# kmkolasinski/tfrecords-reader

Measured on AMD Instinct MI355X. Metric: GiB/s + examples/s device-resident TFRecord->Feature decode, 1/2/4/8 GPU, higher is better.
Workload: dtype u8; 1 GPU; C4 directory (configs[4]) of 256 files, C1-shaped (int64 label + 12 B bytes_list id) records, 524288 +-50 % per file (default_rng(1000+f)), spec CRC-32C; this rank's LPT share (256 files) resident in HBM; records_per_gpu=134295581, framed_bytes_per_gpu=7906235019, parallelism=file-sharded x1 (LPT by bytes, no collective on the data path), batches_per_gpu=4, batch_bytes_max=1976558779, streams=2, tpl_groups_missed=0

## Files before the change

### tfrecords-reader_amd/csrc/tfrg_capi.cpp

```cpp
#include <hip/hip_runtime.h>
#include <stdlib.h>
#include <string.h>

#include <algorithm>
#include <map>
#include <numeric>
#include <string>
#include <unordered_map>
#include <vector>

#include "../../include/tfrg.h"
#include "crc32c.h"
#include "tfrg_dense.h"
#include "tfrg_frame.h"
#include "tfrg_internal.h"
#include "tfrg_learn.h"

namespace tfrg {
void set_error(const std::string& s);

#define HIP_TRY(expr)                                                              \
  do {                                                                             \
    hipError_t e_ = (expr);                                                        \
    if (e_ != hipSuccess) {                                                        \
// ... 27 lines not shown
  template <class T>
  T* as() const {
    return reinterpret_cast<T*>(p);
  }
};

constexpr uint32_t kMissCap = 1u << 16;

}

using namespace tfrg;

struct Offsets {
  const uint64_t* s64 = nullptr;
  const uint64_t* e64 = nullptr;
  const uint32_t* s32 = nullptr;
  const uint32_t* e32 = nullptr;
  uint32_t first = 0;
  uint32_t mode = kOffU64;
};

struct tfrg_ctx {
  int device = 0;
  hipStream_t own_stream = nullptr;
  hipStream_t last_stream = nullptr;
  uint32_t lane_max = 2048;
  uint32_t wave_stage = 0xffffffffu;
  uint64_t record_bound = 0;
  uint64_t call_bound = 0;
  int num_cus = 256;
  uint32_t cu_lds = 65536;
  int tpl_stage = 1;
  uint32_t tpl_gpw = 0;
  DBuf crc_tab, consts;
  DBuf ht, key_hash, key_off, key_blob, key_slot, slot_kind, key_w, krec;
  uint32_t n_keys = 0, n_slots = 0, ht_mask = 0;
  DBuf in_bytes, in_start, in_end;
  DBuf status, aux, verdict, order, count, loc, rs, slot_base, totals, kind_totals;
  DBuf ident;
  size_t ident_n = 0;
  DBuf i64, f32, b_off, b_len, big_list, slow_list, miss, info, tsum, crc_rec, crc_base, crc_part;
  DBuf dq, dq_cnt;
  DBuf lmask, rlist;
  DBuf bdata, boff64, blb, bbig;
  bool materialized = false;
  bool tsum_dirty = true;
  uint32_t info_slot = 0;
  bool info_clean = false;
  uint32_t n = 0;
  uint64_t cap_hint = 0;
  hipEvent_t order_ev = nullptr;
  hipEvent_t dense_ev[2] = {nullptr, nullptr};
  int dense_nt = 0;
  uint64_t nbytes = 0;
  uint64_t cap_i64 = 0, cap_f32 = 0, cap_b = 0;
  bool have_result = false;
  bool rs_complete = false;
  std::unordered_map<std::string, uint32_t> key_id;
  std::vector<int32_t> key_slot_h;
  DBuf tpl;
  uint32_t n_tpl = 0;
  uint32_t tpl_w = 0;
  size_t tpl_img_off = 0;
  uint32_t tpl_img_words = 0;
  uint32_t tpl_tab_words = 0;
  std::vector<uint32_t> tpl_h;
// ... 32 lines not shown
    uint64_t cap_in;
    uint64_t bound;
    uint32_t n, flags;
    hipStream_t st;
  } last{};
  Offsets last_off{};
  uint32_t index_chunk = kIndexChunkDefault;
  DBuf fr_tab, fr_dev;
  void* fr_pin = nullptr;
  size_t fr_pin_cap = 0;
  uint32_t poison[4] = {0xffffffffu, 0xffffffffu, 0xffffffffu, 0xffffffffu};
};

extern "C" {

int tfrg_ctx_create(int device, tfrg_ctx** out) {
  *out = nullptr;
  int ndev = 0;
  HIP_TRY(hipGetDeviceCount(&ndev));
  if (device < 0 || device >= ndev) {
    set_error("bad device index");
    return TFRG_E_ARG;
  }
  HIP_TRY(hipSetDevice(device));
  tfrg_ctx* c = new tfrg_ctx();
  c->device = device;
  if (const char* e = getenv("TFRG_TEMPLATES")) c->tpl_on = atoi(e) != 0;
  if (const char* e = getenv("TFRG_SPEC")) c->spec_on = atoi(e) != 0;
  if (const char* e = getenv("TFRG_TPL_STAGE")) c->tpl_stage = atoi(e);
  if (const char* e = getenv("TFRG_TPL_GPW")) {
    const int v = atoi(e);
    if (v == 2 || v == 4 || v == 8) c->tpl_gpw = (uint32_t)v;
  }
  if (const char* e = getenv("TFRG_OPTIMISTIC")) c->optimistic_on = atoi(e) != 0;
  if (const char* e = getenv("TFRG_WALK_BESIDE")) c->walk_beside = atoi(e) != 0;
  if (const char* e = getenv("TFRG_WALK_BLOCKS")) c->walk_blocks = (uint32_t)atoi(e);
  if (const char* e = getenv("TFRG_DENSE_NT")) c->dense_nt = atoi(e) != 0;
  if (const char* e = getenv("TFRG_DEBUG_POISON_LOC")) {
    char* q = const_cast<char*>(e);
    for (int i = 0; i < 4 && *q; ++i) {
      c->poison[i] = (uint32_t)strtoul(q, &q, 10);
      while (*q == ',' || *q == ' ') ++q;
    }
  }
  hipDeviceProp_t prop;
  if (hipGetDeviceProperties(&prop, device) == hipSuccess) {
    c->num_cus = prop.multiProcessorCount;
    if (prop.maxSharedMemoryPerMultiProcessor) c->cu_lds = (uint32_t)prop.maxSharedMemoryPerMultiProcessor;
  }
  if (hipStreamCreateWithFlags(&c->own_stream, hipStreamNonBlocking) != hipSuccess) {
    delete c;
    set_error("hipStreamCreate failed");
    return TFRG_E_HIP;
  }
  if (hipHostMalloc(reinterpret_cast<void**>(&c->info_pin), (kInfoCount + 8) * 4) != hipSuccess) {
    (void)hipStreamDestroy(c->own_stream);
    delete c;
    set_error("hipHostMalloc failed");
    return TFRG_E_NOMEM;
  }
  std::vector<uint32_t> tab(kCrcTabWords), cst(128);
  CrcTables T;
  crc_make_tables(&T);
  memcpy(tab.data(), T.t, 4096);
  uint32_t M[4][256];
  crc_make_mul_tables(gf_xpow8(1024), M);
// ... 522 lines not shown
  o.loc = c->loc.as<uint2>();
  o.rs = c->rs.as<uint32_t>();
  o.slot_base = c->slot_base.as<uint64_t>();
  o.totals = c->totals.as<uint32_t>();
  o.kind_totals = c->kind_totals.as<uint64_t>();
  o.i64 = c->i64.as<int64_t>();
  o.f32 = c->f32.as<uint32_t>();
  o.b_off = c->b_off.as<uint32_t>();
  o.b_len = c->b_len.as<uint32_t>();
  o.cap_i64 = cap_i64;
  o.cap_f32 = cap_f32;
  o.cap_b = cap_b;
  o.big_list = c->big_list.as<uint32_t>();
  o.miss = c->miss.as<uint32_t>();
  o.miss_cap = kMissCap;
  o.info = info_cur;
  o.info_next = c->info.as<uint32_t>() + (islot ^ 1u) * kInfoCount;
  o.tsum = c->tsum.as<uint32_t>();
  o.tile_stride = tile_stride;
  o.spine_lb = reinterpret_cast<uint64_t*>(o.tsum + (size_t)S * tile_stride);
  o.n_chunks = n_chunks;
  o.irr = o.tsum + (size_t)S * tile_stride + 2ull * S * n_chunks;
  o.slow_list = c->slow_list.as<uint32_t>();
  o.crc_rec = c->crc_rec.as<uint32_t>();
  o.crc_base = c->crc_base.as<uint64_t>();
  o.crc_part = c->crc_part.as<uint64_t>();
  o.lmask = c->lmask.as<uint64_t>();
  o.rlist = c->rlist.as<uint32_t>();
  LaunchCfg cfg;
  cfg.num_cus = c->num_cus;
  cfg.tpl_cu_lds = c->tpl_stage ? c->cu_lds : 0u;
  cfg.tpl_stage_any = c->tpl_stage == 2;
  cfg.tpl_gpw = c->tpl_gpw;
  cfg.lean = c->tpl_on && c->n_tpl;
  cfg.tpl_full = cfg.lean && c->tpl_full;
  cfg.tpl_unchecked = cfg.lean && (c->tpl_frames & 2u) != 0;
  cfg.spec_h = c->spec_h.empty() ? nullptr : c->spec_h.data();
  const uint64_t lane_blocks = (n + 255) / 256;
  const uint64_t lane_cap = (uint64_t)c->num_cus * 8;
  cfg.lane_grid = (int)(lane_blocks < 1 ? 1 : (lane_blocks < lane_cap ? lane_blocks : lane_cap));
  const uint64_t wave_cap = (uint64_t)c->num_cus * 4;
  const uint64_t wave_blocks = (n + 3) / 4;
  cfg.wave_grid = (int)(wave_blocks < 1 ? 1 : (wave_blocks < wave_cap ? wave_blocks : wave_cap));
  cfg.lane_max = c->lane_max;
  cfg.wave_stage = c->wave_stage;
  memcpy(cfg.poison, c->poison, sizeof(cfg.poison));
  cfg.optimistic = c->optimistic_on && !c->no_quiet && c->poison[0] == 0xffffffffu;
  cfg.walk_beside = c->walk_beside;
  cfg.walk_blocks = c->walk_blocks;
  cfg.ran_optimistic = false;
  cfg.ran_quiet_big = false;
  cfg.ord_const = c->ord_const;
  cfg.len_const = c->len_const && !mat;
  cfg.implicit = 0;
  const uint64_t bound = c->call_bound ? c->call_bound : c->record_bound;
  c->call_bound = 0;
  c->last = tfrg_ctx::LastCall{d_bytes, nbytes, cap_in, bound, n, flags, st};
  c->last_off = off;
  o.dq = nullptr;
  o.dq_cnt = nullptr;
  o.dq_blocks = 0;
  cfg.body_count = false;
  if (n && (bound == 0 || bound > c->lane_max)) {
    uint64_t blocks = nbytes >> 18;
    blocks = blocks < 16 ? 16 : (blocks > (1u << 16) ? (1u << 16) : blocks);
    const size_t qb = (size_t)blocks * 64u * kDeferK * 16u, cb = (size_t)blocks * 64u;
// ... 433 lines not shown
```

### tfrecords-reader_amd/csrc/tfrg_decode.cpp

```cpp
#include <algorithm>

#include "../../include/tfrg_status.h"
#include "tfrg_internal.h"

namespace tfrg {

const char* const kStageNames[kNumStages] = {"k_tpl_lane",    "k_lane_count",  "k_body_count", "k_tail_count", "k_spine",
                                             "k_down_gather", "k_tail_gather", "k_bytes"};

static LeanArgs lean_args(const DevBatch& b, const DevSchema& sc, const DevOut& o, const LaunchCfg& cfg,
                          bool placing) {
  const bool nocrc = (b.flags & kFlagNoCrc) != 0;
  LeanArgs a{};
  a.n_tpl = sc.n_tpl;
  a.img_words = sc.tpl_img_words;
  a.tab_words = nocrc ? 0u : sc.tpl_tab_words;
  a.nocrc = nocrc ? 1u : 0u;
  a.strict = (b.flags & kFlagStrictCrc) ? 1u : 0u;
  a.uframes = cfg.tpl_unchecked ? 1u : 0u;
  a.cu_lds = cfg.tpl_cu_lds;
  a.stage_any = cfg.tpl_stage_any ? 1u : 0u;
  a.gpw_force = cfg.tpl_gpw;
  a.lane_max = cfg.lane_max;
  a.tsum = cfg.ran_optimistic ? nullptr : o.tsum;
  a.finish = cfg.ran_optimistic ? sc.slot_kind : nullptr;
  a.implicit = cfg.implicit;
  a.n_slots = sc.n_slots;
  a.tile_stride = o.tile_stride;
  const uint64_t n = b.n;
  for (uint32_t k = 0; k < sc.n_slots; ++k) {
    LeanTgt& t = a.tg[k];
    t.ord = o.order + k * n;
    t.cnt = o.count + k * n;
    t.loc = o.loc + k * n;
    t.rs = o.rs + k * (n + 1);
    const uint32_t sw = placing ? cfg.spec_h[k] : 0u;
    if (!sw) continue;
    const uint32_t kind = sw & 3u;
    const uint64_t base = n * ((sw >> 2) - 1u);
    const uint64_t cap = kind == TFRG_KIND_INT64 ? o.cap_i64 : kind == TFRG_KIND_FLOAT ? o.cap_f32 : o.cap_b;
    t.lim = cap > base ? (uint32_t)std::min<uint64_t>(cap - base, n) : 0u;
    t.kind = kind;
    if (kind == TFRG_KIND_INT64) t.v1 = o.i64 + base;
    else if (kind == TFRG_KIND_FLOAT) t.v1 = o.f32 + base;
    else t.v1 = o.b_off + base;
    t.v2 = o.b_len + base;
  }
  return a;
}

hipError_t launch_decode(const DevBatch& b, const DevSchema& sc, const DevOut& o, LaunchCfg& cfg,
                         const uint32_t* d_tab, const uint32_t* d_consts, hipStream_t st, hipEvent_t* ev) {
  auto mark = [&](int i) {
    if (ev) (void)hipEventRecord(ev[i], st);
  };
// ... 70 lines not shown
```

### tfrecords-reader_amd/csrc/tfrg_internal.h

```cpp
#pragma once
#include <stdint.h>
#include <hip/hip_runtime.h>
#include "tfrg_layout.h"

namespace tfrg {

struct DevSchema {
  uint32_t n_keys;
  uint32_t n_slots;
  uint32_t ht_mask;
  const uint32_t* ht;
  const uint32_t* key_hash;
  const uint32_t* key_off;
  const uint8_t* key_blob;
  const int32_t* key_slot;
  const uint8_t* slot_kind;
  const uint32_t* key_w;
  const uint32_t* krec;
  const uint32_t* tpl;
  const uint32_t* tpl_img;
  uint32_t tpl_img_words;
  uint32_t tpl_tab_words;
  uint32_t n_tpl;
  uint32_t tpl_w;
  const uint32_t* spec;
};

constexpr uint32_t kCrcTabWords = 51200;

struct LeanTgt {
  uint16_t* ord;
  uint32_t* cnt;
  uint2* loc;
  uint32_t* rs;
  void* v1;
  uint32_t* v2;
  uint32_t lim;
  uint32_t kind;
  uint32_t pad[2];
};
struct LeanArgs {
  uint32_t n_tpl;
  uint32_t lane_max;
  uint32_t* tsum;
  uint32_t n_slots;
  uint32_t tile_stride;
  uint32_t img_words;
  uint32_t gpw;
  uint32_t bsplit;
  uint32_t gsplit;
  const uint8_t* finish;
  uint32_t implicit;
  uint32_t tab_words;
  uint32_t cu_lds;
  uint32_t stage_any;
  uint32_t gpw_force;
  uint32_t nocrc;
  uint32_t strict;
  uint32_t uframes;
  LeanTgt tg[kLeanMaxSlots];
};

enum KeyRec : uint32_t { kKrHash = 0, kKrLen, kKrW0, kKrW1, kKrSlot1, kKrSlot2, kKrSlot3, kKrFlags, kKrWords };
constexpr uint32_t kLdsMaxKeys = 256;
constexpr uint32_t kLdsMaxHt = 1024;
inline bool schema_in_lds(const DevSchema& sc) { return sc.n_keys <= kLdsMaxKeys && sc.ht_mask + 1 <= kLdsMaxHt; }

__host__ __device__ inline uint32_t key_hash_words(uint32_t n, uint32_t w0, uint32_t w1) {
  const uint32_t a = (w0 ^ (w0 >> 11) ^ (n << 17)) & 0xffffffu;
  const uint32_t b = (w1 ^ (w1 >> 13) ^ (n << 7)) & 0xffffffu;
#if defined(__HIP_DEVICE_COMPILE__)
  uint32_t p0, p1;
  asm("v_mul_u32_u24 %0, %1, %2" : "=v"(p0) : "v"(a), "v"(0x9E3779u));
  asm("v_mul_u32_u24 %0, %1, %2" : "=v"(p1) : "v"(b), "v"(0x85EBCBu));
  uint32_t h = p0 ^ p1;
#else
  uint32_t h = a * 0x9E3779u;
  h ^= b * 0x85EBCBu;
#endif
  return h ^ (h >> 15);
}

enum OffMode : uint32_t { kOffU64 = 0, kOffU32 = 1, kOffEnds = 2 };

struct DevBatch {
  const uint8_t* bytes;
  uint64_t nbytes;
  const uint64_t* start;
  const uint64_t* end;
// ... 110 lines not shown
  uint64_t* offsets;
  uint64_t offsets_cap;
  uint8_t* data;
  uint64_t data_cap;
  uint64_t* lb;
  uint32_t* ticket;
  uint32_t* big_count;
  uint32_t* big_list;
  uint32_t* overflow;
};
hipError_t launch_materialize(const DevBytes& d, int num_cus, hipStream_t st);
uint64_t materialize_lb_words(uint64_t cap_b);

struct LaunchCfg {
  int num_cus;
  bool lean;
  bool tpl_full;
  bool tpl_unchecked;
  const uint32_t* spec_h;
  int lane_grid;
  int wave_grid;
  uint32_t lane_max;
  uint32_t wave_stage;
  bool body_count;
  uint32_t poison[4];
  bool optimistic;
  bool ran_optimistic;
  bool ord_const;
  bool len_const;
  bool ran_quiet_big;
  uint32_t tpl_cu_lds;
  bool tpl_stage_any;
  uint32_t tpl_gpw;
  bool walk_beside;
  uint32_t walk_blocks;
  uint32_t implicit;
};

enum Stage : int { kStageTplLane = 0, kStageLaneCount, kStageBodyCount, kStageTailCount, kStageSpine,
                   kStageDownGather, kStageTailGather, kStageMaterialize, kNumStages };
extern const char* const kStageNames[kNumStages];

hipError_t launch_tpl_lane(const DevBatch& b, const DevOut& o, const LeanArgs& a, const uint32_t* img, uint32_t w,
                           int num_cus, hipStream_t st);
int lane_count_mode(const DevSchema& sc);
void launch_lane_count(const DevBatch& b, const DevSchema& sc, const DevOut& o, const uint32_t* d_tab,
                       const LaunchCfg& cfg, bool defer_big, int mode, int max_blocks, hipStream_t st);
void launch_body_count(const DevBatch& b, const DevOut& o, int num_cus, hipStream_t st);
bool tail_walk_fits(const DevSchema& sc);
void launch_tail_count(const DevBatch& b, const DevSchema& sc, const DevOut& o, const uint32_t* d_tab,
                       const uint32_t* d_consts, const LaunchCfg& cfg, bool finish, bool walk, uint32_t max_blocks,
                       hipStream_t st);
void launch_poison_loc(const DevOut& o, uint32_t n, uint32_t n_slots, const uint32_t recs[4], hipStream_t st);
void launch_spine(const DevOut& o, const DevSchema& sc, uint32_t n_tiles, uint32_t n, hipStream_t st);
void launch_down_gather(const DevBatch& b, const DevSchema& sc, const DevOut& o, const LaunchCfg& cfg,
                        uint32_t n_tiles, uint32_t resident, hipStream_t st);
void launch_tail_gather(const DevBatch& b, const DevSchema& sc, const DevOut& o, const LaunchCfg& cfg, int max_blocks,
                        hipStream_t st);
hipError_t launch_fill_placed_rows(uint32_t* rs, const uint32_t* info, uint32_t n_slots, uint32_t n, hipStream_t st);
hipError_t launch_stream_read(const void* d, uint64_t nbytes, uint32_t* sink, hipStream_t st, int variant);
struct FrTab;
hipError_t launch_frame_index(const FrTab& T, int num_cus, hipStream_t st);
hipError_t launch_decode(const DevBatch& b, const DevSchema& sc, const DevOut& o, LaunchCfg& cfg,
                         const uint32_t* d_crc_tables, const uint32_t* d_wave_consts, hipStream_t stream,
                         hipEvent_t* ev);

// ... 2 lines not shown
```

### tfrecords-reader_amd/csrc/tfrg_layout.h

```cpp
#pragma once
#include <stdint.h>

namespace tfrg {

constexpr uint32_t kTplMaxL = 240, kTplMaxEntries = 16;
constexpr uint32_t kLtMaxW = 64;
constexpr uint32_t kLeanMaxSlots = 16;
constexpr uint32_t kLtL = 0, kLtNe = 1, kLtCrcw = 2, kLtChain = 3, kLtK = 4, kLtAbsent = 5, kLtFrame = 6, kLtEnt = 8,
                   kLtWin = kLtEnt + 4 * kTplMaxEntries, kLtSlot = kLtWin + 3 * kLtMaxW,
                   kLtWords = kLtSlot + 3 * kLeanMaxSlots;

constexpr uint32_t kLiPtabWords = 4 * 256;
constexpr uint32_t kTplSample = 4096;
constexpr uint32_t kTplMaxLane = 32;
constexpr uint32_t kLiHdr = 8, kLiSlotQ = kLiHdr, kLiLut = kLiSlotQ + kLeanMaxSlots,
                   kLiLutWords = (kTplMaxL + 1 + 3) / 4, kLiTpl = (kLiLut + kLiLutWords + 3) & ~3u;
constexpr uint32_t kLiQValue = 1u << 16, kLiQSingle = 1u << 17;
constexpr uint32_t kLiTw(uint32_t W) { return 4 + 3 * W + 4 * kLeanMaxSlots; }
constexpr uint32_t kLiMaxWords = (65536u - 32768u - 512u) / 4u;

constexpr uint32_t kCountInline = 0x80000000u;

}
```

### tfrecords-reader_amd/csrc/tfrg_tpl.hip

```cpp
#include <hip/hip_runtime.h>
#include "tfrg_internal.h"
#include "tfrg_dev.h"
#include "crc32c.h"
#include "../../include/tfrg_status.h"

namespace tfrg {

namespace {

constexpr int kTplBlock = 512;
constexpr uint32_t kTplTabWords = 8;
static_assert(4u * kTplTabWords * kLiPtabWords + 4u * kLiMaxWords + 512u <= 65536u, "lane image + CRC tables exceed LDS");
constexpr uint32_t kStageWords = 1024 + 32, kStageRounds = (kStageWords * 4u + 1023u) / 1024u;
constexpr uint32_t kStTimgWords = (53248u - 64u - (kTplBlock / 64u) * kStageWords * 4u) / 16u * 4u;
template <bool ST>
__device__ __forceinline__ uint32_t* st_timg() {
  if constexpr (ST) {
    __shared__ __attribute__((aligned(16))) uint32_t s_timg[kStTimgWords];
    return s_timg;
  } else {
    return nullptr;
  }
}
template <bool ST>
__device__ __forceinline__ uint32_t* st_stage() {
  if constexpr (ST) {
    __shared__ __attribute__((aligned(16))) uint32_t s_stage[(kTplBlock / 64u) * kStageWords];
    return s_stage;
  } else {
    return nullptr;
  }
}
constexpr uint32_t kHitVerdict = TFRG_V_LEN_MATCH | TFRG_V_LEN_CRC | TFRG_V_DATA_CRC;

typedef __attribute__((address_space(4))) const uint32_t cu32;
typedef __attribute__((address_space(3))) void lds_void;
#ifndef TFRG_TPL_SPAN_AUX
#define TFRG_TPL_SPAN_AUX 2
#endif
#ifndef TFRG_TPL_STORE_NT
#define TFRG_TPL_STORE_NT 1
#endif
template <int Q>
__device__ __forceinline__ uint32_t tl(const uint8_t* tw, uint32_t bx) {
  return *reinterpret_cast<const uint32_t*>(tw + Q * 1024 + bx);
}

__device__ __forceinline__ uint32_t lin_word(const uint8_t* tw, uint32_t x) {
  return xor3(tl<3>(tw, byte_x4<0>(x)), tl<2>(tw, byte_x4<1>(x)), tl<1>(tw, byte_x4<2>(x))) ^ tl<0>(tw, byte_x4<3>(x));
}

typedef uint32_t u32x4 __attribute__((ext_vector_type(4)));

struct LaneOff {
  uint32_t s, e;
};

__device__ __forceinline__ uint32_t wave_sum(uint32_t x) {
#pragma unroll
  for (int m = 1; m < 64; m <<= 1) x += (uint32_t)__shfl_xor((int)x, m, 64);
  return x;
}

__device__ void tpl_quiet_finish(const DevOut& o, const uint8_t* slot_kind, uint32_t n_slots, uint32_t n,
                                 uint32_t listed) {
  if (threadIdx.x < kInfoCount) o.info_next[threadIdx.x] = 0u;
  if (listed != 0u) return;
  all_placed_finish(o, slot_kind, n_slots, n, kTplBlock);
}

template <int W, int OM, bool ST, bool UF>
__global__ __launch_bounds__(kTplBlock, W == 16 ? 6 : (W == 32 ? 4 : 2)) void k_tpl_lane(
    DevBatch B, DevOut o, LeanArgs A, const uint32_t* __restrict__ img, const uint32_t* __restrict__ tabs) {
  static_assert(W == 16 || W == 32 || W == 64, "window words");
  static_assert(!ST || W == 16, "staged windows: W = 16");
  typedef uint32_t wvec __attribute__((ext_vector_type(W)));
  extern __shared__ __attribute__((aligned(16))) uint32_t dyn_lds[];
  uint32_t* tab = dyn_lds;
  if constexpr (ST) tab = st_timg<ST>();
  uint32_t* const limg = tab + A.tab_words;
  constexpr uint32_t kWaves = kTplBlock / 64;
  constexpr uint32_t kTw = kLiTw(W);
  const uint32_t lane = threadIdx.x & 63u, wib = rfl32(threadIdx.x >> 6);
  cu32* gimg = (cu32*)img;
  const bool nocrc = UF && A.nocrc;
  const uint32_t crcw_u = nocrc ? 0u : gimg[3], chain_u = nocrc ? (uint32_t)W : gimg[4];
  auto tabw = [&](uint32_t j) -> const uint8_t* {
    return reinterpret_cast<const uint8_t*>(tab) + 4u * kLiPtabWords * ((gimg[6u + (j >> 2)] >> (8u * (j & 3u))) & 0xffu);
  };
  const uint8_t* lut = reinterpret_cast<const uint8_t*>(limg + kLiLut);
  const __amdgpu_buffer_rsrc_t rsrc =
      __builtin_amdgcn_make_buffer_rsrc(const_cast<uint8_t*>(B.bytes), (short)0, (int)(uint32_t)B.nbytes, 0x00020000);
  const uint32_t nb = (uint32_t)B.nbytes;
  const uint32_t ngroups = (B.n + 63u) >> 6;
  static_assert(kTileShift == 8, "4 groups of 64 records per tile");
  const bool tail = blockIdx.x >= A.bsplit;
  const uint32_t gpw = tail ? 2u : A.gpw;
  const uint32_t gbeg0 = tail ? A.gsplit + ((blockIdx.x - A.bsplit) * kWaves + wib) * 2u : (blockIdx.x * kWaves + wib) * gpw;
  const uint32_t gbeg = gbeg0 < ngroups ? gbeg0 : ngroups;
  const uint32_t gend = gbeg + gpw < ngroups ? gbeg + gpw : ngroups;
  const bool whole = (gpw & 3u) == 0u;

  auto offsets = [&](uint32_t g) -> LaneOff {
    LaneOff f{1u, 0u};
    const uint32_t r = (g << 6) + lane;
    if (g < gend && r < B.n) {
      if constexpr (OM == kOffU64) {
        const uint64_t s = B.start[r], e = B.end[r];
        if (((s | e) >> 32) == 0) f = LaneOff{(uint32_t)s, (uint32_t)e};
      } else if constexpr (OM == kOffU32) {
        f = LaneOff{B.start32[r], B.end32[r]};
      } else {
        f.e = B.end32[r];
        f.s = lane ? 0u : (r ? B.end32[r - 1] : B.first);
      }
    }
    return f;
  };
  auto start_of = [&](const LaneOff& f) -> uint32_t {
    if constexpr (OM == kOffEnds)
      return (uint32_t)__builtin_amdgcn_update_dpp((int)f.s, (int)f.e, 0x138, 0xf, 0xf, false);
    else
      return f.s;
  };
  auto in_batch = [&](uint32_t g, uint32_t s, uint32_t e) {
    return (g << 6) + lane < B.n && s <= e && e <= nb && e >= 16u;
  };
  auto window = [&](wvec& wn, const LaneOff& f) {
    const uint32_t e = f.e;
    const bool full = e >= 4u * W && e <= nb;
    const uint32_t voff = full ? e - 4u * W : 0xffffff00u;
#pragma unroll
    for (int q = 0; q < W / 4; ++q) {
      const u32x4 v = __builtin_bit_cast(u32x4, __builtin_amdgcn_raw_buffer_load_b128(rsrc, voff + 16u * q, 0, 0));
      wn[4 * q] = v.x;
      wn[4 * q + 1] = v.y;
      wn[4 * q + 2] = v.z;
      wn[4 * q + 3] = v.w;
    }
  };
  struct Span {
    uint32_t lo;
    bool on;
  };
  auto fill = [&](const LaneOff& f, uint32_t g) -> Span {
    if constexpr (ST) {
      uint32_t* const stg = st_stage<ST>() + wib * kStageWords;
      const uint32_t e = f.e;
      const uint32_t g0 = g << 6;
      const uint32_t nv = g < gend ? (B.n - g0 < 64u ? B.n - g0 : 64u) : 0u;
      const uint32_t pe = (uint32_t)__builtin_amdgcn_update_dpp((int)e, (int)e, 0x138, 0xf, 0xf, false);
      const bool bad = lane < nv && (e < pe || e > nb);
      if (nv && !__ballot(bad)) {
        const uint32_t e0 = rfl32(e), hi = (uint32_t)__builtin_amdgcn_readlane((int)e, (int)(nv - 1u));
        const uint32_t lo = (e0 >= 4u * W ? e0 - 4u * W : 0u) & ~15u;
        const uint32_t nch = (hi - lo + 15u) >> 4;
        if (hi > lo && nch * 16u + 4u <= kStageWords * 4u && lo + nch * 16u <= nb) {
#pragma unroll
          for (uint32_t k = 0; k < kStageRounds; ++k)
            if (lane + 64u * k < nch)
              __builtin_amdgcn_raw_ptr_buffer_load_lds(rsrc, (lds_void*)(stg + 256u * k), 16, lo + 16u * (lane + 64u * k), 0,
                                                       0, TFRG_TPL_SPAN_AUX);
          return Span{lo, true};
        }
      }
    }
    return Span{0u, false};
  };
  auto take = [&](wvec& wn, const LaneOff& f, uint32_t g, const Span& sp_) {
    if constexpr (ST) {
      if (sp_.on) {
        const uint32_t* const stg = st_stage<ST>() + wib * kStageWords;
        const uint32_t e = f.e;
        const bool full = e >= 4u * W && (g << 6) + lane < B.n;
        const uint32_t b0 = full ? e - 4u * W - sp_.lo : 0u;
        const uint32_t* const sp = stg + (b0 >> 2);
        const uint32_t sh = b0 & 3u;
        uint32_t prev = sp[0];
#pragma unroll
        for (int i = 0; i < W; ++i) {
          const uint32_t nx = sp[i + 1];
          wn[i] = __builtin_amdgcn_alignbyte(nx, prev, sh);
          prev = nx;
        }
        if (__ballot(!full)) {
#pragma unroll
          for (int i = 0; i < W; ++i) wn[i] = full ? wn[i] : 0u;
        }
        return;
      }
    }
    window(wn, f);
    if constexpr (ST) __builtin_amdgcn_s_waitcnt(0x0F70);
  };
  auto head_fix = [&](wvec& wn, const LaneOff& f, uint32_t g) {
    if (g != 0u) return;
    const uint32_t e = f.e;
    const bool full = e >= 4u * W && e <= nb;
    const bool head = in_batch(g, start_of(f), e) && !full;
    if (__ballot(head)) {
#pragma unroll
      for (int i = 0; i < W; ++i) {
        uint32_t x = 0;
#pragma unroll
        for (int b = 0; b < 4; ++b) {
          const int64_t p = (int64_t)e - 4 * W + 4 * i + b;
          if (head && p >= 0) x |= (uint32_t)__builtin_amdgcn_raw_buffer_load_b8(rsrc, (uint32_t)p, 0, 0) << (8 * b);
        }
        if (head) wn[i] = x;
      }
      if constexpr (ST) __builtin_amdgcn_s_waitcnt(0x0F70);
    }
  };
  auto wsel = [](const wvec& w, uint32_t q) -> uint32_t {
    if constexpr (W <= 32) {
      return w[q & (W - 1u)];
    } else {
      uint32_t a = 0;
#pragma unroll
      for (int i = 0; i < W; ++i)
        if (q == (uint32_t)i) a = w[i];
      return a;
    }
  };
  uint32_t acc = 0;
  uint32_t listed = 0;
  auto proc = [&](const wvec& w, uint32_t g, const LaneOff& f) {
    const uint32_t r = (g << 6) + lane;
    const bool valid = r < B.n;
    const uint32_t st = start_of(f), en = f.e;
    const bool inb = in_batch(g, st, en);
    const uint32_t rl = en - st;
    uint32_t cand = inb && rl >= 16u && rl - 16u <= kTplMaxL && rl <= A.lane_max ? (uint32_t)lut[rl - 16u] : 0xffu;
    uint32_t tsel = 0xffu;
    while (__ballot(cand != 0xffu)) {
      const bool act = cand != 0xffu;
      const uint32_t* tp = limg + kLiTpl + (act ? cand : 0u) * kTw;
      const u32x4 meta = *reinterpret_cast<const u32x4*>(tp);
      uint32_t diff = 0;
#pragma unroll
      for (int q = 0; q < W / 4; ++q) {
        const u32x4 bm = *reinterpret_cast<const u32x4*>(tp + 4 + 4 * q);
        const u32x4 mm = *reinterpret_cast<const u32x4*>(tp + 4 + W + 4 * q);
        diff |= ((w[4 * q] ^ bm.x) & mm.x) | ((w[4 * q + 1] ^ bm.y) & mm.y) | ((w[4 * q + 2] ^ bm.z) & mm.z) |
                ((w[4 * q + 3] ^ bm.w) & mm.w);
        if (q & 1) __builtin_amdgcn_sched_barrier(0);
      }
      const uint32_t* cm = tp + 4 + 2 * W;
      uint32_t c = 0;
      if (chain_u < (uint32_t)(W - 9)) {
#pragma unroll
        for (int i = 0; i < W - 9; ++i)
          if ((uint32_t)i >= chain_u) c = lin_word(tabw(7), c ^ (w[i] & cm[i]));
      }
      uint32_t lin = 0;
#define TFRG_LIN(j)                                                                                       \
  if (crcw_u & (1u << (j))) lin ^= lin_word(tabw(j), (w[W - 9 + (j)] & cm[W - 9 + (j)]) ^ ((j) == 0 ? c : 0u));
      TFRG_LIN(0) TFRG_LIN(1) TFRG_LIN(2) TFRG_LIN(3) TFRG_LIN(4) TFRG_LIN(5) TFRG_LIN(6) TFRG_LIN(7)
#undef TFRG_LIN
      bool ok = act && diff == 0u;
      if constexpr (UF) {
        const uint32_t mc = crc_mask(lin ^ meta.y);
        ok = ok && (nocrc || (meta.w ? mc != 0u && !A.strict : mc == w[W - 1]));
      } else {
        ok = ok && crc_mask(lin ^ meta.y) == w[W - 1];
      }
      tsel = ok ? cand : tsel;
      cand = act && !ok ? meta.z : 0xffu;
    }
    const bool hit = tsel != 0xffu;
    if (hit && !(A.implicit & TFRG_IMPLICIT_STATUS)) {
      o.status[r] = TFRG_OK;
      if constexpr (UF)
        o.verdict[r] = (uint8_t)(nocrc || limg[kLiTpl + tsel * kTw + 3] ? (uint32_t)TFRG_V_LEN_MATCH : kHitVerdict);
      else
        o.verdict[r] = (uint8_t)kHitVerdict;
    }
    if (__ballot(hit)) {
      const uint32_t* ts = limg + kLiTpl + (hit ? tsel : 0u) * kTw + 4 + 3 * W;
      for (uint32_t k = 0; k < A.n_slots; ++k) {
        const uint32_t sq = gimg[kLiSlotQ + k];
        const u32x4 z = *reinterpret_cast<const u32x4*>(ts + 4u * k);
        const uint32_t mode = z.x & 0xffu, len = (z.x >> 8) & 0xffu, pos = z.y, cw = z.z;
        uint32_t lx = pos, ly = len;
        if (sq & kLiQValue) {
          const uint32_t qw = pos >> 2;
          uint32_t a = 0, b = 0;
          for (uint32_t i = sq & 0xffu; i <= ((sq >> 8) & 0xffu); ++i) {
            const bool at = qw == i;
            a = at ? wsel(w, i) : a;
            b = at ? wsel(w, i + 1u) : b;
          }
          const uint32_t x = __builtin_amdgcn_alignbyte(b, a, pos & 3u);
          if (mode == 1u || mode == 2u) {
            lx = mode == 1u ? vgroups(x, bytes_mask(len)) : x;
            ly = 0;
          }
        }
        if (mode == 3u) lx = en + pos;
        const uint32_t tot = !A.tsum ? 0u
                             : (sq & kLiQSingle) ? (uint32_t)__popcll(__ballot(hit && cw != 0u))
// ... 6 lines not shown
              constexpr bool kNt = ST && TFRG_TPL_STORE_NT;
              if (T.kind == TFRG_KIND_INT64) {
                st_nt<kNt>(reinterpret_cast<uint64_t*>(T.v1) + r, (uint64_t)lx);
              } else {
                st_nt<kNt>(reinterpret_cast<uint32_t*>(T.v1) + r, lx);
                if (T.kind == TFRG_KIND_BYTES && !(A.implicit & TFRG_IMPLICIT_BYTES_LEN)) st_nt<kNt>(T.v2 + r, ly);
              }
            }
          } else {
            T.cnt[r] = cw;
            T.loc[r] = make_uint2(lx, ly);
          }
        }
        acc += lane == k ? tot : 0u;
      }
    }
    const uint64_t mm = __ballot(valid && !hit);
    if (lane == 0) {
      o.lmask[g] = mm;
      if (mm) o.rlist[atomicAdd(&o.info[kInfoResid], 1u)] = g;
    }
    listed += mm ? 1u : 0u;
  };
  auto flush = [&](uint32_t g) {
    if (lane < A.n_slots && acc && A.tsum) {
      if (whole)
        A.tsum[lane * A.tile_stride + (g >> 2)] = acc;
      else
        atomicAdd(&A.tsum[lane * A.tile_stride + (g >> 2)], acc);
    }
    acc = 0;
  };
  LaneOff fa = offsets(gbeg), f0 = offsets(gbeg + 1u);
  static_assert(kTplTabWords * kLiPtabWords % (4u * kTplBlock) == 0u, "table copy in whole 16-byte rounds");
  constexpr uint32_t kTabRounds = kTplTabWords * kLiPtabWords / (4u * kTplBlock);
  const uint32_t tab16 = A.tab_words >> 2;
  u32x4 tv[kTabRounds];
#pragma unroll
  for (uint32_t j = 0; j < kTabRounds; ++j)
    if (threadIdx.x + j * kTplBlock < tab16) tv[j] = reinterpret_cast<const u32x4*>(tabs)[threadIdx.x + j * kTplBlock];
  const uint32_t iw0 = threadIdx.x < A.img_words ? img[threadIdx.x] : 0u;
  wvec wa;
  Span sa{0u, false};
  if constexpr (ST)
    sa = fill(fa, gbeg);
  else
    window(wa, fa);
#pragma unroll
  for (uint32_t j = 0; j < kTabRounds; ++j)
    if (threadIdx.x + j * kTplBlock < tab16) reinterpret_cast<u32x4*>(tab)[threadIdx.x + j * kTplBlock] = tv[j];
  if (threadIdx.x < A.img_words) limg[threadIdx.x] = iw0;
  for (uint32_t i = threadIdx.x + kTplBlock; i < A.img_words; i += kTplBlock) limg[i] = img[i];
  __syncthreads();
  if constexpr (ST) {
    for (uint32_t g = gbeg; g < gend; ++g) {
      asm volatile("" ::: "memory");
      __builtin_amdgcn_s_waitcnt(0x0F70);
      asm volatile("" ::: "memory");
      take(wa, fa, g, sa);
      asm volatile("" ::: "memory");
      __builtin_amdgcn_s_waitcnt(0xC07F);
      asm volatile("" ::: "memory");
      Span sn{0u, false};
      if (g + 1u < gend) sn = fill(f0, g + 1u);
      const LaneOff f2 = offsets(g + 2u);
      head_fix(wa, fa, g);
      proc(wa, g, fa);
      if (((g + 1u) & 3u) == 0u || g + 1u >= gend) flush(g);
      fa = f0;
      f0 = f2;
      sa = sn;
    }
  } else {
    for (uint32_t g = gbeg; g < gend; ++g) {
      head_fix(wa, fa, g);
      proc(wa, g, fa);
      if (((g + 1u) & 3u) == 0u || g + 1u >= gend) flush(g);
      if (g + 1u < gend) {
        window(wa, f0);
        fa = f0;
        f0 = offsets(g + 2u);
      }
    }
  }
  if (A.finish) {
    __shared__ uint32_t s_listed[kWaves];
    __shared__ uint32_t s_last, s_total;
    if (lane == 0) s_listed[wib] = listed;
    __syncthreads();
    if (threadIdx.x == 0) {
      uint32_t mine = 0;
      for (uint32_t i = 0; i < kWaves; ++i) mine += s_listed[i];
      const uint64_t old = atomicAdd(reinterpret_cast<unsigned long long*>(o.info + kInfoTplDone),
                                     ((unsigned long long)mine << 32) | 1ull);
      s_last = (uint32_t)old == gridDim.x - 1u;
      s_total = (uint32_t)(old >> 32) + mine;
    }
    __syncthreads();
    if (s_last) tpl_quiet_finish(o, A.finish, A.n_slots, B.n, s_total);
  }
}

}

hipError_t launch_tpl_lane(const DevBatch& b, const DevOut& o, const LeanArgs& a, const uint32_t* img, uint32_t w,
                           int num_cus, hipStream_t st) {
  const uint32_t groups = (b.n + 63u) / 64u;
  const uint32_t tiles = (groups + 3u) / 4u;
  const uint32_t need = (tiles + kTplBlock / 64 - 1) / (kTplBlock / 64);
  LeanArgs a2 = a;
  a2.gpw = need < (uint32_t)num_cus / 2u ? 1u : need < (uint32_t)num_cus ? 2u : need >= 8u * (uint32_t)num_cus ? 8u : 4u;
  const bool forced = a.gpw_force == 2u || a.gpw_force == 4u || a.gpw_force == 8u;
  if (forced) a2.gpw = a.gpw_force;
  static const bool split_on = [] {
    const char* e = getenv("TFRG_TPL_TAIL");
    return !e || atoi(e) != 0;
  }();
  constexpr uint32_t kW = kTplBlock / 64;
  uint32_t gsplit = groups, bsplit = 0xffffffffu;
  if (split_on && !forced && a2.gpw == 8u) {
    const uint32_t small = 3u * (uint32_t)num_cus * kW * 2u;
    if (groups > 4u * small) {
      const uint32_t big_blocks = (groups - small) / (kW * a2.gpw);
      gsplit = big_blocks * kW * a2.gpw;
      bsplit = big_blocks;
    }
  }
  a2.gsplit = gsplit;
  a2.bsplit = bsplit;
  const uint32_t blocks = bsplit != 0xffffffffu
                              ? bsplit + (groups - gsplit + kW * 2u - 1u) / (kW * 2u)
                              : ((groups + a2.gpw - 1u) / a2.gpw + kW - 1u) / kW;
  const dim3 grid(blocks ? blocks : 1u);
  const uint32_t* tabs = img + a.img_words;
  size_t lds = ((size_t)a.tab_words + a.img_words) * 4;
  constexpr size_t lds_st = ((size_t)kStTimgWords + kW * kStageWords) * 4;
  static_assert(lds_st + 64u <= 65536u, "staged kernel's LDS");
  const bool staged = w == 16 && (a2.gpw >= 8u || a.stage_any) && (size_t)a.tab_words + a.img_words <= kStTimgWords &&
                      3u * ((lds_st + 64u + 2047u) & ~(size_t)2047u) <= a.cu_lds;
  if (staged) lds = 0;
  const bool uf = a.nocrc || a.uframes;
#define TFRG_TPL_LAUNCH(WW, OO, SS)                                                                            \
  if (uf) hipLaunchKernelGGL((k_tpl_lane<WW, OO, SS, true>), grid, dim3(kTplBlock), lds, st, b, o, a2, img, tabs); \
  else hipLaunchKernelGGL((k_tpl_lane<WW, OO, SS, false>), grid, dim3(kTplBlock), lds, st, b, o, a2, img, tabs)
#define TFRG_TPL_OM(WW, SS)                                                    \
  switch (b.omode) {                                                           \
    case kOffU64: TFRG_TPL_LAUNCH(WW, kOffU64, SS); break;                     \
    case kOffU32: TFRG_TPL_LAUNCH(WW, kOffU32, SS); break;                     \
    default: TFRG_TPL_LAUNCH(WW, kOffEnds, SS); break;                         \
  }
  switch (w) {
    case 16:
      if (staged) {
        TFRG_TPL_OM(16, true)
      } else {
        TFRG_TPL_OM(16, false)
      }
      break;
    case 32: TFRG_TPL_OM(32, false) break;
    case 64: TFRG_TPL_OM(64, false) break;
    default: return hipErrorInvalidValue;
  }
#undef TFRG_TPL_OM
#undef TFRG_TPL_LAUNCH
  return hipGetLastError();
}

}
```

Measured before the change: 4255 GiB/s.

## Add wide staged template-lane kernel variant with larger workgroups and split match loop

```diff
diff --git a/tfrecords-reader_amd/csrc/tfrg_capi.cpp b/tfrecords-reader_amd/csrc/tfrg_capi.cpp
--- a/tfrecords-reader_amd/csrc/tfrg_capi.cpp
+++ b/tfrecords-reader_amd/csrc/tfrg_capi.cpp
@@ -83,6 +83,7 @@
   uint32_t cu_lds = 65536;
   int tpl_stage = 1;
   uint32_t tpl_gpw = 0;
+  uint32_t tpl_wide = 1;
   DBuf crc_tab, consts;
   DBuf ht, key_hash, key_off, key_blob, key_slot, slot_kind, key_w, krec;
   uint32_t n_keys = 0, n_slots = 0, ht_mask = 0;
@@ -181,6 +182,10 @@
     const int v = atoi(e);
     if (v == 2 || v == 4 || v == 8) c->tpl_gpw = (uint32_t)v;
   }
+  if (const char* e = getenv("TFRG_TPL_WIDE")) {
+    const int v = atoi(e);
+    if (v >= 0 && v <= 2) c->tpl_wide = (uint32_t)v;
+  }
   if (const char* e = getenv("TFRG_OPTIMISTIC")) c->optimistic_on = atoi(e) != 0;
   if (const char* e = getenv("TFRG_WALK_BESIDE")) c->walk_beside = atoi(e) != 0;
   if (const char* e = getenv("TFRG_WALK_BLOCKS")) c->walk_blocks = (uint32_t)atoi(e);
@@ -769,6 +774,7 @@
   cfg.tpl_cu_lds = c->tpl_stage ? c->cu_lds : 0u;
   cfg.tpl_stage_any = c->tpl_stage == 2;
   cfg.tpl_gpw = c->tpl_gpw;
+  cfg.tpl_wide = c->tpl_wide;
   cfg.lean = c->tpl_on && c->n_tpl;
   cfg.tpl_full = cfg.lean && c->tpl_full;
   cfg.tpl_unchecked = cfg.lean && (c->tpl_frames & 2u) != 0;
diff --git a/tfrecords-reader_amd/csrc/tfrg_decode.cpp b/tfrecords-reader_amd/csrc/tfrg_decode.cpp
--- a/tfrecords-reader_amd/csrc/tfrg_decode.cpp
+++ b/tfrecords-reader_amd/csrc/tfrg_decode.cpp
@@ -21,6 +21,7 @@
   a.cu_lds = cfg.tpl_cu_lds;
   a.stage_any = cfg.tpl_stage_any ? 1u : 0u;
   a.gpw_force = cfg.tpl_gpw;
+  a.wide = cfg.tpl_wide;
   a.lane_max = cfg.lane_max;
   a.tsum = cfg.ran_optimistic ? nullptr : o.tsum;
   a.finish = cfg.ran_optimistic ? sc.slot_kind : nullptr;
diff --git a/tfrecords-reader_amd/csrc/tfrg_internal.h b/tfrecords-reader_amd/csrc/tfrg_internal.h
--- a/tfrecords-reader_amd/csrc/tfrg_internal.h
+++ b/tfrecords-reader_amd/csrc/tfrg_internal.h
@@ -55,6 +55,7 @@
   uint32_t cu_lds;
   uint32_t stage_any;
   uint32_t gpw_force;
+  uint32_t wide;
   uint32_t nocrc;
   uint32_t strict;
   uint32_t uframes;
@@ -231,6 +232,7 @@
   uint32_t tpl_cu_lds;
   bool tpl_stage_any;
   uint32_t tpl_gpw;
+  uint32_t tpl_wide;
   bool walk_beside;
   uint32_t walk_blocks;
   uint32_t implicit;
diff --git a/tfrecords-reader_amd/csrc/tfrg_layout.h b/tfrecords-reader_amd/csrc/tfrg_layout.h
--- a/tfrecords-reader_amd/csrc/tfrg_layout.h
+++ b/tfrecords-reader_amd/csrc/tfrg_layout.h
@@ -19,6 +19,35 @@
 constexpr uint32_t kLiTw(uint32_t W) { return 4 + 3 * W + 4 * kLeanMaxSlots; }
 constexpr uint32_t kLiMaxWords = (65536u - 32768u - 512u) / 4u;
 
+#ifndef TFRG_TPL_WIDE_NW
+#define TFRG_TPL_WIDE_NW 11
+#endif
+constexpr uint32_t kTplWideWaves = TFRG_TPL_WIDE_NW;
+static_assert(kTplWideWaves == 11 || kTplWideWaves == 16, "the wide staged workgroup: 11 x 2 or 16 x 1 per CU");
+constexpr uint32_t kTplStageWords = 1024 + 32;
+constexpr uint32_t kTplCuLds = 163840;
+constexpr uint32_t kTplStageWgs(uint32_t nw) { return nw <= 8 ? 3u : nw < 16 ? 2u : 1u; }
+constexpr uint32_t kTplStaticOther(uint32_t nw) { return (8u + 4u * nw + 63u) & ~63u; }
+constexpr uint32_t kTplTimgWords(uint32_t nw) {
+  return ((kTplCuLds / kTplStageWgs(nw) & ~2047u) - kTplStaticOther(nw) - nw * kTplStageWords * 4u) / 16u * 4u;
+}
+static_assert(kTplTimgWords(8) * 4u == 19392u && kTplTimgWords(11) * 4u == 35392u && kTplTimgWords(16) * 4u == 96128u,
+              "staged budgets");
+constexpr uint32_t kTplStagedLds(uint32_t nw) {
+  return (kTplTimgWords(nw) + nw * kTplStageWords) * 4u + kTplStaticOther(nw);
+}
+enum TplVariant : uint32_t { kTplPerLane = 0, kTplStaged8 = 1, kTplStagedWide = 2 };
+constexpr TplVariant tpl_variant(uint32_t w, uint32_t tab_words, uint32_t img_words, uint32_t gpw, bool stage_any,
+                                 uint32_t cu_lds, uint32_t wide) {
+  if (w != 16u || !(gpw >= 8u || stage_any)) return kTplPerLane;
+  const uint64_t need = (uint64_t)tab_words + img_words;
+  const bool fit8 = need <= kTplTimgWords(8) && kTplStageWgs(8) * ((kTplStagedLds(8) + 2047u) & ~2047u) <= cu_lds;
+  const bool fitw = wide != 0u && need <= kTplTimgWords(kTplWideWaves) &&
+                    kTplStageWgs(kTplWideWaves) * ((kTplStagedLds(kTplWideWaves) + 2047u) & ~2047u) <= cu_lds;
+  if (wide == 2u && fitw) return kTplStagedWide;
+  return fit8 ? kTplStaged8 : fitw ? kTplStagedWide : kTplPerLane;
+}
+
 constexpr uint32_t kCountInline = 0x80000000u;
 
 }
diff --git a/tfrecords-reader_amd/csrc/tfrg_tpl.hip b/tfrecords-reader_amd/csrc/tfrg_tpl.hip
--- a/tfrecords-reader_amd/csrc/tfrg_tpl.hip
+++ b/tfrecords-reader_amd/csrc/tfrg_tpl.hip
@@ -11,21 +11,20 @@
 constexpr int kTplBlock = 512;
 constexpr uint32_t kTplTabWords = 8;
 static_assert(4u * kTplTabWords * kLiPtabWords + 4u * kLiMaxWords + 512u <= 65536u, "lane image + CRC tables exceed LDS");
-constexpr uint32_t kStageWords = 1024 + 32, kStageRounds = (kStageWords * 4u + 1023u) / 1024u;
-constexpr uint32_t kStTimgWords = (53248u - 64u - (kTplBlock / 64u) * kStageWords * 4u) / 16u * 4u;
-template <bool ST>
+constexpr uint32_t kStageWords = kTplStageWords, kStageRounds = (kStageWords * 4u + 1023u) / 1024u;
+template <bool ST, int NW>
 __device__ __forceinline__ uint32_t* st_timg() {
   if constexpr (ST) {
-    __shared__ __attribute__((aligned(16))) uint32_t s_timg[kStTimgWords];
+    __shared__ __attribute__((aligned(16))) uint32_t s_timg[kTplTimgWords(NW)];
     return s_timg;
   } else {
     return nullptr;
   }
 }
-template <bool ST>
+template <bool ST, int NW>
 __device__ __forceinline__ uint32_t* st_stage() {
   if constexpr (ST) {
-    __shared__ __attribute__((aligned(16))) uint32_t s_stage[(kTplBlock / 64u) * kStageWords];
+    __shared__ __attribute__((aligned(16))) uint32_t s_stage[NW * kStageWords];
     return s_stage;
   } else {
     return nullptr;
@@ -63,23 +62,25 @@
 }
 
 __device__ void tpl_quiet_finish(const DevOut& o, const uint8_t* slot_kind, uint32_t n_slots, uint32_t n,
-                                 uint32_t listed) {
+                                 uint32_t listed, uint32_t blk) {
   if (threadIdx.x < kInfoCount) o.info_next[threadIdx.x] = 0u;
   if (listed != 0u) return;
-  all_placed_finish(o, slot_kind, n_slots, n, kTplBlock);
-}
-
-template <int W, int OM, bool ST, bool UF>
-__global__ __launch_bounds__(kTplBlock, W == 16 ? 6 : (W == 32 ? 4 : 2)) void k_tpl_lane(
+  all_placed_finish(o, slot_kind, n_slots, n, blk);
+}
+
+template <int W, int OM, bool ST, bool UF, int NW = kTplBlock / 64>
+__global__ __launch_bounds__(NW * 64, NW == 16 ? 4 : W == 16 ? 6 : (W == 32 ? 4 : 2)) void k_tpl_lane(
     DevBatch B, DevOut o, LeanArgs A, const uint32_t* __restrict__ img, const uint32_t* __restrict__ tabs) {
   static_assert(W == 16 || W == 32 || W == 64, "window words");
   static_assert(!ST || W == 16, "staged windows: W = 16");
+  static_assert(NW * 64 == kTplBlock || ST, "workgroups of another size: the staged kernel's");
+  constexpr uint32_t kBlock = NW * 64;
   typedef uint32_t wvec __attribute__((ext_vector_type(W)));
   extern __shared__ __attribute__((aligned(16))) uint32_t dyn_lds[];
   uint32_t* tab = dyn_lds;
-  if constexpr (ST) tab = st_timg<ST>();
+  if constexpr (ST) tab = st_timg<ST, NW>();
   uint32_t* const limg = tab + A.tab_words;
-  constexpr uint32_t kWaves = kTplBlock / 64;
+  constexpr uint32_t kWaves = NW;
   constexpr uint32_t kTw = kLiTw(W);
   const uint32_t lane = threadIdx.x & 63u, wib = rfl32(threadIdx.x >> 6);
   cu32* gimg = (cu32*)img;
@@ -145,7 +146,7 @@
   };
   auto fill = [&](const LaneOff& f, uint32_t g) -> Span {
     if constexpr (ST) {
-      uint32_t* const stg = st_stage<ST>() + wib * kStageWords;
+      uint32_t* const stg = st_stage<ST, NW>() + wib * kStageWords;
       const uint32_t e = f.e;
       const uint32_t g0 = g << 6;
       const uint32_t nv = g < gend ? (B.n - g0 < 64u ? B.n - g0 : 64u) : 0u;
@@ -170,7 +171,7 @@
   auto take = [&](wvec& wn, const LaneOff& f, uint32_t g, const Span& sp_) {
     if constexpr (ST) {
       if (sp_.on) {
-        const uint32_t* const stg = st_stage<ST>() + wib * kStageWords;
+        const uint32_t* const stg = st_stage<ST, NW>() + wib * kStageWords;
         const uint32_t e = f.e;
         const bool full = e >= 4u * W && (g << 6) + lane < B.n;
         const uint32_t b0 = full ? e - 4u * W - sp_.lo : 0u;
@@ -233,40 +234,93 @@
     const uint32_t rl = en - st;
     uint32_t cand = inb && rl >= 16u && rl - 16u <= kTplMaxL && rl <= A.lane_max ? (uint32_t)lut[rl - 16u] : 0xffu;
     uint32_t tsel = 0xffu;
-    while (__ballot(cand != 0xffu)) {
-      const bool act = cand != 0xffu;
-      const uint32_t* tp = limg + kLiTpl + (act ? cand : 0u) * kTw;
-      const u32x4 meta = *reinterpret_cast<const u32x4*>(tp);
-      uint32_t diff = 0;
-#pragma unroll
-      for (int q = 0; q < W / 4; ++q) {
-        const u32x4 bm = *reinterpret_cast<const u32x4*>(tp + 4 + 4 * q);
-        const u32x4 mm = *reinterpret_cast<const u32x4*>(tp + 4 + W + 4 * q);
-        diff |= ((w[4 * q] ^ bm.x) & mm.x) | ((w[4 * q + 1] ^ bm.y) & mm.y) | ((w[4 * q + 2] ^ bm.z) & mm.z) |
-                ((w[4 * q + 3] ^ bm.w) & mm.w);
-        if (q & 1) __builtin_amdgcn_sched_barrier(0);
-      }
-      const uint32_t* cm = tp + 4 + 2 * W;
-      uint32_t c = 0;
-      if (chain_u < (uint32_t)(W - 9)) {
-#pragma unroll
-        for (int i = 0; i < W - 9; ++i)
-          if ((uint32_t)i >= chain_u) c = lin_word(tabw(7), c ^ (w[i] & cm[i]));
-      }
-      uint32_t lin = 0;
+    if constexpr (NW * 64 == kTplBlock) {
+      while (__ballot(cand != 0xffu)) {
+        const bool act = cand != 0xffu;
+        const uint32_t* tp = limg + kLiTpl + (act ? cand : 0u) * kTw;
+        const u32x4 meta = *reinterpret_cast<const u32x4*>(tp);
+        uint32_t diff = 0;
+#pragma unroll
+        for (int q = 0; q < W / 4; ++q) {
+          const u32x4 bm = *reinterpret_cast<const u32x4*>(tp + 4 + 4 * q);
+          const u32x4 mm = *reinterpret_cast<const u32x4*>(tp + 4 + W + 4 * q);
+          diff |= ((w[4 * q] ^ bm.x) & mm.x) | ((w[4 * q + 1] ^ bm.y) & mm.y) | ((w[4 * q + 2] ^ bm.z) & mm.z) |
+                  ((w[4 * q + 3] ^ bm.w) & mm.w);
+          if (q & 1) __builtin_amdgcn_sched_barrier(0);
+        }
+        const uint32_t* cm = tp + 4 + 2 * W;
+        uint32_t c = 0;
+        if (chain_u < (uint32_t)(W - 9)) {
+#pragma unroll
+          for (int i = 0; i < W - 9; ++i)
+            if ((uint32_t)i >= chain_u) c = lin_word(tabw(7), c ^ (w[i] & cm[i]));
+        }
+        uint32_t lin = 0;
 #define TFRG_LIN(j)                                                                                       \
-  if (crcw_u & (1u << (j))) lin ^= lin_word(tabw(j), (w[W - 9 + (j)] & cm[W - 9 + (j)]) ^ ((j) == 0 ? c : 0u));
-      TFRG_LIN(0) TFRG_LIN(1) TFRG_LIN(2) TFRG_LIN(3) TFRG_LIN(4) TFRG_LIN(5) TFRG_LIN(6) TFRG_LIN(7)
+    if (crcw_u & (1u << (j))) lin ^= lin_word(tabw(j), (w[W - 9 + (j)] & cm[W - 9 + (j)]) ^ ((j) == 0 ? c : 0u));
+        TFRG_LIN(0) TFRG_LIN(1) TFRG_LIN(2) TFRG_LIN(3) TFRG_LIN(4) TFRG_LIN(5) TFRG_LIN(6) TFRG_LIN(7)
 #undef TFRG_LIN
-      bool ok = act && diff == 0u;
-      if constexpr (UF) {
-        const uint32_t mc = crc_mask(lin ^ meta.y);
-        ok = ok && (nocrc || (meta.w ? mc != 0u && !A.strict : mc == w[W - 1]));
-      } else {
-        ok = ok && crc_mask(lin ^ meta.y) == w[W - 1];
-      }
-      tsel = ok ? cand : tsel;
-      cand = act && !ok ? meta.z : 0xffu;
+        bool ok = act && diff == 0u;
+        if constexpr (UF) {
+          const uint32_t mc = crc_mask(lin ^ meta.y);
+          ok = ok && (nocrc || (meta.w ? mc != 0u && !A.strict : mc == w[W - 1]));
+        } else {
+          ok = ok && crc_mask(lin ^ meta.y) == w[W - 1];
+        }
+        tsel = ok ? cand : tsel;
+        cand = act && !ok ? meta.z : 0xffu;
+      }
+    } else {
+      auto tpl_diff = [&](const uint32_t* tp) -> uint32_t {
+        uint32_t diff = 0;
+#pragma unroll
+        for (int q = 0; q < W / 4; ++q) {
+          const u32x4 tb = *reinterpret_cast<const u32x4*>(tp + 4 + 4 * q);
+          const u32x4 tm = *reinterpret_cast<const u32x4*>(tp + 4 + W + 4 * q);
+          diff |= ((w[4 * q] ^ tb.x) & tm.x) | ((w[4 * q + 1] ^ tb.y) & tm.y) | ((w[4 * q + 2] ^ tb.z) & tm.z) |
+                  ((w[4 * q + 3] ^ tb.w) & tm.w);
+          if (q & 1) __builtin_amdgcn_sched_barrier(0);
+        }
+        return diff;
+      };
+      auto tpl_crc = [&](const uint32_t* tp, const u32x4& meta, bool ok) -> bool {
+        const uint32_t* cm = tp + 4 + 2 * W;
+        uint32_t c = 0;
+        if (chain_u < (uint32_t)(W - 9)) {
+#pragma unroll
+          for (int i = 0; i < W - 9; ++i)
+            if ((uint32_t)i >= chain_u) c = lin_word(tabw(7), c ^ (w[i] & cm[i]));
+        }
+        uint32_t lin = 0;
+#define TFRG_LIN(j)                                                                                       \
+    if (crcw_u & (1u << (j))) lin ^= lin_word(tabw(j), (w[W - 9 + (j)] & cm[W - 9 + (j)]) ^ ((j) == 0 ? c : 0u));
+        TFRG_LIN(0) TFRG_LIN(1) TFRG_LIN(2) TFRG_LIN(3) TFRG_LIN(4) TFRG_LIN(5) TFRG_LIN(6) TFRG_LIN(7)
+#undef TFRG_LIN
+        if constexpr (UF) {
+          const uint32_t mc = crc_mask(lin ^ meta.y);
+          ok = ok && (nocrc || (meta.w ? mc != 0u && !A.strict : mc == w[W - 1]));
+        } else {
+          ok = ok && crc_mask(lin ^ meta.y) == w[W - 1];
+        }
+        return ok;
+      };
+      while (__ballot(cand != 0xffu)) {
+        uint32_t sel = 0xffu;
+        while (__ballot(cand != 0xffu && sel == 0xffu)) {
+          const bool act = cand != 0xffu && sel == 0xffu;
+          const uint32_t* tp = limg + kLiTpl + (act ? cand : 0u) * kTw;
+          const uint32_t nxt = tp[2];
+          const uint32_t diff = tpl_diff(tp);
+          sel = act && diff == 0u ? cand : sel;
+          cand = act && diff != 0u ? nxt : cand;
+        }
+        const bool act = sel != 0xffu;
+        const uint32_t* tp = limg + kLiTpl + (act ? sel : 0u) * kTw;
+        const u32x4 meta = *reinterpret_cast<const u32x4*>(tp);
+        const bool ok = tpl_crc(tp, meta, act);
+        tsel = ok ? sel : tsel;
+        cand = act && !ok ? meta.z : 0xffu;
+      }
     }
     const bool hit = tsel != 0xffu;
     if (hit && !(A.implicit & TFRG_IMPLICIT_STATUS)) {
@@ -339,13 +393,13 @@
     acc = 0;
   };
   LaneOff fa = offsets(gbeg), f0 = offsets(gbeg + 1u);
-  static_assert(kTplTabWords * kLiPtabWords % (4u * kTplBlock) == 0u, "table copy in whole 16-byte rounds");
-  constexpr uint32_t kTabRounds = kTplTabWords * kLiPtabWords / (4u * kTplBlock);
+  static_assert(kTplTabWords * kLiPtabWords % (4u * kTplBlock) == 0u, "8 waves: the table copy in whole 16-byte rounds");
+  constexpr uint32_t kTabRounds = (kTplTabWords * kLiPtabWords + 4u * kBlock - 1u) / (4u * kBlock);
   const uint32_t tab16 = A.tab_words >> 2;
   u32x4 tv[kTabRounds];
 #pragma unroll
   for (uint32_t j = 0; j < kTabRounds; ++j)
-    if (threadIdx.x + j * kTplBlock < tab16) tv[j] = reinterpret_cast<const u32x4*>(tabs)[threadIdx.x + j * kTplBlock];
+    if (threadIdx.x + j * kBlock < tab16) tv[j] = reinterpret_cast<const u32x4*>(tabs)[threadIdx.x + j * kBlock];
   const uint32_t iw0 = threadIdx.x < A.img_words ? img[threadIdx.x] : 0u;
   wvec wa;
   Span sa{0u, false};
@@ -355,9 +409,9 @@
     window(wa, fa);
 #pragma unroll
   for (uint32_t j = 0; j < kTabRounds; ++j)
-    if (threadIdx.x + j * kTplBlock < tab16) reinterpret_cast<u32x4*>(tab)[threadIdx.x + j * kTplBlock] = tv[j];
+    if (threadIdx.x + j * kBlock < tab16) reinterpret_cast<u32x4*>(tab)[threadIdx.x + j * kBlock] = tv[j];
   if (threadIdx.x < A.img_words) limg[threadIdx.x] = iw0;
-  for (uint32_t i = threadIdx.x + kTplBlock; i < A.img_words; i += kTplBlock) limg[i] = img[i];
+  for (uint32_t i = threadIdx.x + kBlock; i < A.img_words; i += kBlock) limg[i] = img[i];
   __syncthreads();
   if constexpr (ST) {
     for (uint32_t g = gbeg; g < gend; ++g) {
@@ -404,7 +458,7 @@
       s_total = (uint32_t)(old >> 32) + mine;
     }
     __syncthreads();
-    if (s_last) tpl_quiet_finish(o, A.finish, A.n_slots, B.n, s_total);
+    if (s_last) tpl_quiet_finish(o, A.finish, A.n_slots, B.n, s_total, kBlock);
   }
 }
 
@@ -423,10 +477,12 @@
     const char* e = getenv("TFRG_TPL_TAIL");
     return !e || atoi(e) != 0;
   }();
-  constexpr uint32_t kW = kTplBlock / 64;
+  static_assert(kTplStagedLds(kTplBlock / 64) <= 65536u, "staged kernel's LDS");
+  const TplVariant var = tpl_variant(w, a.tab_words, a.img_words, a2.gpw, a.stage_any != 0u, a.cu_lds, a.wide);
+  const uint32_t kW = var == kTplStagedWide ? kTplWideWaves : (uint32_t)kTplBlock / 64u;
   uint32_t gsplit = groups, bsplit = 0xffffffffu;
   if (split_on && !forced && a2.gpw == 8u) {
-    const uint32_t small = 3u * (uint32_t)num_cus * kW * 2u;
+    const uint32_t small = (var == kTplStagedWide ? kTplStageWgs(kTplWideWaves) : 3u) * (uint32_t)num_cus * kW * 2u;
     if (groups > 4u * small) {
       const uint32_t big_blocks = (groups - small) / (kW * a2.gpw);
       gsplit = big_blocks * kW * a2.gpw;
@@ -440,32 +496,29 @@
                               : ((groups + a2.gpw - 1u) / a2.gpw + kW - 1u) / kW;
   const dim3 grid(blocks ? blocks : 1u);
   const uint32_t* tabs = img + a.img_words;
-  size_t lds = ((size_t)a.tab_words + a.img_words) * 4;
-  constexpr size_t lds_st = ((size_t)kStTimgWords + kW * kStageWords) * 4;
-  static_assert(lds_st + 64u <= 65536u, "staged kernel's LDS");
-  const bool staged = w == 16 && (a2.gpw >= 8u || a.stage_any) && (size_t)a.tab_words + a.img_words <= kStTimgWords &&
-                      3u * ((lds_st + 64u + 2047u) & ~(size_t)2047u) <= a.cu_lds;
-  if (staged) lds = 0;
+  const size_t lds = var == kTplPerLane ? ((size_t)a.tab_words + a.img_words) * 4 : 0;
   const bool uf = a.nocrc || a.uframes;
-#define TFRG_TPL_LAUNCH(WW, OO, SS)                                                                            \
-  if (uf) hipLaunchKernelGGL((k_tpl_lane<WW, OO, SS, true>), grid, dim3(kTplBlock), lds, st, b, o, a2, img, tabs); \
-  else hipLaunchKernelGGL((k_tpl_lane<WW, OO, SS, false>), grid, dim3(kTplBlock), lds, st, b, o, a2, img, tabs)
-#define TFRG_TPL_OM(WW, SS)                                                    \
+#define TFRG_TPL_LAUNCH(WW, OO, SS, NN)                                                                                \
+  if (uf) hipLaunchKernelGGL((k_tpl_lane<WW, OO, SS, true, NN>), grid, dim3(NN * 64), lds, st, b, o, a2, img, tabs); \
+  else hipLaunchKernelGGL((k_tpl_lane<WW, OO, SS, false, NN>), grid, dim3(NN * 64), lds, st, b, o, a2, img, tabs)
+#define TFRG_TPL_OM(WW, SS, NN)                                                \
   switch (b.omode) {                                                           \
-    case kOffU64: TFRG_TPL_LAUNCH(WW, kOffU64, SS); break;                     \
-    case kOffU32: TFRG_TPL_LAUNCH(WW, kOffU32, SS); break;                     \
-    default: TFRG_TPL_LAUNCH(WW, kOffEnds, SS); break;                         \
+    case kOffU64: TFRG_TPL_LAUNCH(WW, kOffU64, SS, NN); break;                 \
+    case kOffU32: TFRG_TPL_LAUNCH(WW, kOffU32, SS, NN); break;                 \
+    default: TFRG_TPL_LAUNCH(WW, kOffEnds, SS, NN); break;                     \
   }
   switch (w) {
     case 16:
-      if (staged) {
-        TFRG_TPL_OM(16, true)
+      if (var == kTplStagedWide) {
+        TFRG_TPL_OM(16, true, kTplWideWaves)
+      } else if (var == kTplStaged8) {
+        TFRG_TPL_OM(16, true, kTplBlock / 64)
       } else {
-        TFRG_TPL_OM(16, false)
+        TFRG_TPL_OM(16, false, kTplBlock / 64)
       }
       break;
-    case 32: TFRG_TPL_OM(32, false) break;
-    case 64: TFRG_TPL_OM(64, false) break;
+    case 32: TFRG_TPL_OM(32, false, kTplBlock / 64) break;
+    case 64: TFRG_TPL_OM(64, false, kTplBlock / 64) break;
     default: return hipErrorInvalidValue;
   }
 #undef TFRG_TPL_OM
```

Measured after the change: 4167 GiB/s. 0.979x the previous value.
